# metagentools/VStrains

Measured on AMD Instinct MI355X. Metric: PE read pairs/sec through PE-link inference (GFA index + packed reads in HBM -> node_mat/short_mat), higher is better.
Workload: dtype u32

## Files before the change

### include/vstrains_hip.h

```cpp
#ifndef VSTRAINS_HIP_H
#define VSTRAINS_HIP_H

#include <stddef.h>
#include <stdint.h>

#ifdef __cplusplus
extern "C" {
#endif

#define VS_ABI_VERSION 10

enum {
    VS_OK = 0,
    VS_E_ARG = -1,
    VS_E_HIP = -2,
    VS_E_OOM = -3,
    VS_E_NODE_BASE = -4,
    VS_E_STATE = -5,
    VS_E_RANGE = -6,
    VS_E_UTF8 = -7,
    VS_E_KEY = -8,
    VS_E_FPE = -9,
    VS_E_RECURSION = -10
};
// ... 63 lines not shown
int vs_bgzf_shard_plan(const uint32_t *counts, uint64_t n_members, int no_final_newline, uint64_t first, uint64_t last, uint64_t plan[3]);
int vs_fastq_stream_open_range(vs_ctx *ctx, const char *fwd_path, const char *rve_path, const uint64_t range[6], uint64_t n_pairs,
                               vs_fastq_stream **out);

int vs_write_matrix_text(vs_ctx *ctx, const char *path, const uint8_t *ids, const uint64_t *id_off,
                         uint32_t n, const int64_t *mat);

int vs_synth_pairs(vs_ctx *ctx, const uint8_t *genomes, const uint64_t *goff,
                   const uint32_t *cum, uint32_t n_strains, uint64_t seed, uint64_t first_pair,
                   uint64_t n_pairs, uint32_t read_len, uint32_t sub_thresh, uint32_t n_thresh,
                   vs_reads **out);

int vs_pe_count(vs_ctx *ctx, const vs_reads *reads, uint32_t *d_node_mat, uint32_t *d_short_mat,
                uint64_t *d_stats);

int vs_pe_count_tracked(vs_ctx *ctx, const vs_reads *reads, uint32_t *d_node_mat, uint32_t *d_short_mat,
                        uint64_t *d_stats, uint8_t *d_tile_map);
int vs_counts_zero_tracked(vs_ctx *ctx, uint32_t *d_node_mat, uint32_t *d_short_mat, uint32_t n, uint8_t *d_tile_map);

int vs_counts_fold(vs_ctx *ctx, uint32_t *d_counts, int64_t *d_wide, uint64_t n);

int vs_counts_occupied(vs_ctx *ctx, const void *d_cells, uint32_t cell_bytes, uint64_t n_stretches, uint8_t *d_occ);

int vs_comm_unique_id(vs_ctx *ctx, uint8_t id[128]);
int vs_comm_init_rank(vs_ctx *ctx, int n_ranks, const uint8_t id[128], int rank, void **comm);
int vs_comm_destroy(vs_ctx *ctx, void *comm);
int vs_pe_allreduce(vs_ctx *ctx, void *comm, void *d_node_mat, void *d_short_mat, uint64_t *d_stats,
                    uint32_t n, int wide);

int vs_pe_map_ends(vs_ctx *ctx, const vs_reads *reads, uint32_t cap, uint32_t *lists,
                   uint32_t *counts);

int vs_pe_last_timing(vs_ctx *ctx, double ms[5]);
const char *vs_pe_last_kernel(const vs_ctx *ctx);
enum {
    VS_RAN_LOCUS_LDS_SORT = 1,
    VS_RAN_LOCUS_GLOBAL_SORT = 2,
    VS_RAN_PE_MID = 8,
    VS_RAN_ROW_OWNERS = 16
};
uint32_t vs_pe_last_launched(const vs_ctx *ctx);

typedef struct vs_links vs_links;
int vs_links_from_counts(vs_ctx *ctx, const uint32_t *d_node_mat, const uint32_t *d_short_mat,
                         uint32_t n, vs_links **out);
int vs_links_from_counts_tracked(vs_ctx *ctx, const uint32_t *d_node_mat, const uint32_t *d_short_mat, uint32_t n,
                                 const uint8_t *d_tile_map, uint32_t sparse_min_nodes, vs_links **out);
int vs_links_from_wide(vs_ctx *ctx, const int64_t *d_node_mat, const int64_t *d_short_mat,
                       uint32_t n, vs_links **out);
int vs_links_from_host(vs_ctx *ctx, const int64_t *node_mat, const int64_t *short_mat, uint32_t n,
                       vs_links **out);
int vs_links_reserve(vs_ctx *ctx, uint32_t n);
void vs_links_free(vs_ctx *ctx, vs_links *links);
int vs_links_size(const vs_links *links, uint32_t *n);
int vs_links_to_host(vs_ctx *ctx, const vs_links *links, int64_t *out );
int vs_links_block_sums(vs_ctx *ctx, const vs_links *links, const uint64_t *list_off,
                        const uint32_t *list_idx, uint32_t n_lists, const uint32_t *qa,
                        const uint32_t *qb, uint64_t n_queries, int64_t *out);
int vs_links_group_matrix(vs_ctx *ctx, const vs_links *links, const uint64_t *list_off,
                          const uint32_t *list_idx, uint32_t n_groups, int64_t *out);

int vs_graph_refresh(vs_ctx *ctx, uint32_t n_vertices, uint32_t n_edge_slots,
                     const uint64_t *row_ptr, const uint32_t *n_out, const uint32_t *nbr,
                     const uint32_t *eidx, const double *dp, const uint8_t *vertex_black,
                     const uint8_t *edge_black, double *flow, uint8_t *nontrivial,
                     uint8_t *fork_kind, int32_t *chain_next, int32_t *chain_top,
// ... 46 lines not shown
```

### vstrains_amd/_native.py

```python
from __future__ import annotations

import ctypes as C
import os

_HERE = os.path.dirname(os.path.abspath(__file__))
LIB_PATH = os.path.join(_HERE, "libvstrains_hip.so")

VS_OK = 0
VS_E_ARG, VS_E_HIP, VS_E_OOM, VS_E_NODE_BASE, VS_E_STATE, VS_E_RANGE, VS_E_UTF8, VS_E_KEY, VS_E_FPE = -1, -2, -3, -4, -5, -6, -7, -8, -9

SYMBOLS = {
    "vs_abi_version": (C.c_int, []),
    "vs_device_count": (C.c_int, []),
    "vs_ctx_create": (C.c_int, [C.c_int, C.POINTER(C.c_void_p)]),
    "vs_ctx_destroy": (None, [C.c_void_p]),
    "vs_last_error": (C.c_char_p, [C.c_void_p]),
    "vs_ctx_set_stream": (C.c_int, [C.c_void_p, C.c_void_p]),
    "vs_ctx_sync": (C.c_int, [C.c_void_p]),
    "vs_index_build": (C.c_int, [C.c_void_p, C.c_void_p, C.c_void_p, C.c_uint32, C.c_uint32,
                                 C.POINTER(C.c_uint32), C.POINTER(C.c_uint8)]),
    "vs_index_info": (C.c_int, [C.c_void_p, C.POINTER(C.c_uint64)]),
    "vs_index_export": (C.c_int, [C.c_void_p, C.c_void_p, C.c_void_p, C.c_void_p, C.c_void_p, C.c_void_p, C.POINTER(C.c_uint64)]),
    "vs_node_order_host": (C.c_int, [C.c_void_p, C.c_void_p, C.c_uint32, C.c_uint32, C.c_void_p]),
    "vs_reads_pack": (C.c_int, [C.c_void_p, C.c_void_p, C.c_void_p, C.c_uint64, C.POINTER(C.c_void_p)]),
# ... 13 lines not shown
    "vs_fastq_block": (C.c_int, [C.c_void_p, C.c_void_p, C.c_uint64, C.c_uint64, C.POINTER(C.c_void_p)]),
    "vs_fastq_stream_open": (C.c_int, [C.c_void_p, C.c_char_p, C.c_char_p, C.POINTER(C.c_void_p)]),
    "vs_fastq_stream_next": (C.c_int, [C.c_void_p, C.c_void_p, C.c_uint64, C.POINTER(C.c_void_p), C.POINTER(C.c_uint64)]),
    "vs_fastq_stream_info": (C.c_int, [C.c_void_p, C.POINTER(C.c_uint64)]),
    "vs_fastq_stream_close": (None, [C.c_void_p]),
    "vs_fastq_scan_text": (C.c_int, [C.c_void_p, C.c_void_p, C.c_uint64, C.c_uint32, C.c_void_p, C.c_uint64, C.POINTER(C.c_uint64)]),
    "vs_bgzf_walk": (C.c_int, [C.c_void_p, C.c_uint64, C.c_void_p, C.c_uint64, C.POINTER(C.c_uint64)]),
    "vs_inflate_host": (C.c_int, [C.c_void_p, C.c_uint32, C.c_void_p, C.c_uint32, C.c_uint32, C.POINTER(C.c_uint32)]),
    "vs_inflate_bgzf": (C.c_int, [C.c_void_p, C.c_void_p, C.c_uint64, C.c_void_p, C.c_uint64, C.c_uint32, C.c_void_p, C.c_uint64,
                                  C.POINTER(C.c_uint64)]),
    "vs_fastq_stream_inflate_info": (C.c_int, [C.c_void_p, C.POINTER(C.c_uint64)]),
    "vs_bgzf_walk_file": (C.c_int, [C.c_char_p, C.c_void_p, C.c_uint64, C.POINTER(C.c_uint64)]),
    "vs_bgzf_count_lines": (C.c_int, [C.c_void_p, C.c_char_p, C.c_void_p, C.c_uint64, C.c_void_p, C.POINTER(C.c_uint64)]),
    "vs_inflate_count_host": (C.c_int, [C.c_void_p, C.c_uint32, C.c_uint32, C.c_uint32, C.POINTER(C.c_uint32)]),
    "vs_bgzf_shard_plan": (C.c_int, [C.c_void_p, C.c_uint64, C.c_int, C.c_uint64, C.c_uint64, C.POINTER(C.c_uint64)]),
    "vs_fastq_stream_open_range": (C.c_int, [C.c_void_p, C.c_char_p, C.c_char_p, C.POINTER(C.c_uint64), C.c_uint64, C.POINTER(C.c_void_p)]),
    "vs_write_matrix_text": (C.c_int, [C.c_void_p, C.c_char_p, C.c_void_p, C.c_void_p, C.c_uint32, C.c_void_p]),
    "vs_synth_pairs": (C.c_int, [C.c_void_p, C.c_void_p, C.c_void_p, C.c_void_p, C.c_uint32, C.c_uint64,
                                 C.c_uint64, C.c_uint64, C.c_uint32, C.c_uint32, C.c_uint32,
                                 C.POINTER(C.c_void_p)]),
    "vs_pe_count": (C.c_int, [C.c_void_p, C.c_void_p, C.c_void_p, C.c_void_p, C.c_void_p]),
    "vs_pe_count_tracked": (C.c_int, [C.c_void_p, C.c_void_p, C.c_void_p, C.c_void_p, C.c_void_p, C.c_void_p]),
    "vs_counts_zero_tracked": (C.c_int, [C.c_void_p, C.c_void_p, C.c_void_p, C.c_uint32, C.c_void_p]),
    "vs_counts_fold": (C.c_int, [C.c_void_p, C.c_void_p, C.c_void_p, C.c_uint64]),
    "vs_counts_occupied": (C.c_int, [C.c_void_p, C.c_void_p, C.c_uint32, C.c_uint64, C.c_void_p]),
    "vs_comm_unique_id": (C.c_int, [C.c_void_p, C.c_void_p]),
    "vs_comm_init_rank": (C.c_int, [C.c_void_p, C.c_int, C.c_void_p, C.c_int, C.POINTER(C.c_void_p)]),
    "vs_comm_destroy": (C.c_int, [C.c_void_p, C.c_void_p]),
    "vs_pe_allreduce": (C.c_int, [C.c_void_p, C.c_void_p, C.c_void_p, C.c_void_p, C.c_void_p, C.c_uint32, C.c_int]),
    "vs_pe_map_ends": (C.c_int, [C.c_void_p, C.c_void_p, C.c_uint32, C.c_void_p, C.c_void_p]),
    "vs_pe_last_kernel": (C.c_char_p, [C.c_void_p]),
    "vs_pe_last_launched": (C.c_uint32, [C.c_void_p]),
    "vs_pe_last_timing": (C.c_int, [C.c_void_p, C.POINTER(C.c_double)]),
    "vs_links_from_counts": (C.c_int, [C.c_void_p, C.c_void_p, C.c_void_p, C.c_uint32, C.POINTER(C.c_void_p)]),
    "vs_links_from_counts_tracked": (C.c_int, [C.c_void_p, C.c_void_p, C.c_void_p, C.c_uint32, C.c_void_p, C.c_uint32, C.POINTER(C.c_void_p)]),
    "vs_links_from_wide": (C.c_int, [C.c_void_p, C.c_void_p, C.c_void_p, C.c_uint32, C.POINTER(C.c_void_p)]),
    "vs_links_from_host": (C.c_int, [C.c_void_p, C.c_void_p, C.c_void_p, C.c_uint32, C.POINTER(C.c_void_p)]),
    "vs_links_reserve": (C.c_int, [C.c_void_p, C.c_uint32]),
    "vs_links_free": (None, [C.c_void_p, C.c_void_p]),
    "vs_links_size": (C.c_int, [C.c_void_p, C.POINTER(C.c_uint32)]),
    "vs_links_to_host": (C.c_int, [C.c_void_p, C.c_void_p, C.c_void_p]),
    "vs_links_block_sums": (C.c_int, [C.c_void_p, C.c_void_p, C.c_void_p, C.c_void_p, C.c_uint32, C.c_void_p,
                                      C.c_void_p, C.c_uint64, C.c_void_p]),
    "vs_links_group_matrix": (C.c_int, [C.c_void_p, C.c_void_p, C.c_void_p, C.c_void_p, C.c_uint32, C.c_void_p]),
    "vs_graph_refresh": (C.c_int, [C.c_void_p, C.c_uint32, C.c_uint32] + [C.c_void_p] * 13 + [C.POINTER(C.c_uint32)]),
    "vs_stage_create": (C.c_int, [C.c_void_p, C.c_void_p, C.POINTER(C.c_void_p)]),
    "vs_dev_alloc": (C.c_int, [C.c_void_p, C.c_size_t, C.POINTER(C.c_void_p)]),
    "vs_dev_free": (C.c_int, [C.c_void_p, C.c_void_p]),
    "vs_dev_zero": (C.c_int, [C.c_void_p, C.c_void_p, C.c_size_t]),
    "vs_dev_to_host": (C.c_int, [C.c_void_p, C.c_void_p, C.c_void_p, C.c_size_t]),
}

_lib = None


class NativeError(RuntimeError):
    def __init__(self, code: int, msg: str):
        super().__init__("libvstrains_hip: %s (code %d)" % (msg, code))
        self.code = code


def lib():
    global _lib
    if _lib is None:
        if not os.path.exists(LIB_PATH):
            raise ImportError(
# ... 20 lines not shown
```

### vstrains_amd/csrc/vs_internal.h

```cpp
#pragma once

#include <hip/hip_runtime.h>
#include <stdint.h>
#include <string>
#include <vector>

#include "../../include/vstrains_hip.h"
#include "vs_buf.h"
#include "vs_pe_plan.h"

#define VS_WAVE 64
#define VS_PAD_WORDS 16


struct VsNodeMeta {
    uint32_t woff;
    uint32_t len;
};

struct VsSlot {
    uint64_t key;
    uint32_t a;
    uint32_t b;
};
// ... 46 lines not shown
    const uint32_t *inv4;
};
#define VS_FLAG_N 1u
#define VS_FLAG_INVALID 2u
#define VS_FLAG_MANY 4u
#define VS_LEN_MASK 0x00FFFFFFu

struct FqStage {
    VsPinnedBuf words, woff, meta;
    hipEvent_t done = nullptr;
    bool in_flight = false;
};

void vs_tuning_load(VsTuning &t, bool experiment);

struct vs_ctx {
    int device = 0;
    bool experiment = false;
    VsTuning tune;
    hipStream_t stream = nullptr;
    std::string err;
    FqStage fq_stage[2];
    unsigned fq_next = 0;
    bool has_index = false;
    VsIndexDev idx{};
    VsDevBuf d_meta, d_fwd, d_table, d_post;
    uint64_t n_seed_pos = 0, n_slots = 0, n_distinct = 0, index_bytes = 0;
    uint32_t max_node_len = 0;
    VsDevBuf d_slow_list;
    VsDevBuf d_slow_count;
    enum SlowCount : uint32_t {
        SC_MID = 0,
        SC_ACC_QUEUE = 1,
        SC_SLOW = 8,
        SC_STRIP_QUEUE = 9,
        SC_OWNERS = 15,
        SC_WORDS = 16
    };
    VsDevBuf links_spare;
    uint32_t links_spare_n = 0;
    VsDevBuf d_slow_list2;
    VsDevBuf d_dense;
    uint32_t dense_nodes = 0xFFFFFFFFu;
    VsDevBuf d_locus_keys, d_perm, d_locus_hist, d_scan_tmp;
    double last_sort_ms = 0;
    VsDevBuf d_lists, d_list_counts;
    VsDevBuf d_rows, d_row_entries, d_mult, d_ltab;
    VsDevBuf scratch[32];
    struct CachedBuf { VsDevBuf buf; bool used; };
    std::vector<CachedBuf> cache;
    hipEvent_t ev[5] = {nullptr, nullptr, nullptr, nullptr, nullptr};
    double last_ms[3] = {0, 0, 0};
    const char *last_kernel = "";
    uint32_t last_launched = 0;
    int n_cu = 256;
};

struct vs_reads {
    uint64_t n_ends = 0, n_words = 0, max_len = 0, n_invalid = 0, bytes = 0;
    void *d_woff = nullptr, *d_meta = nullptr, *d_words = nullptr, *d_mask = nullptr, *d_inv4 = nullptr;
    bool cached = false;
    VsDevBuf own[5];
    unsigned n_own = 0;
    hipError_t own_alloc(void *&view, size_t bytes) {
        const hipError_t e = own[n_own].reserve(bytes);
        view = own[n_own].ptr();
// ... 131 lines not shown
```

### vstrains_amd/csrc/vs_pe.hip

```cpp
#include <stdio.h>
#include <stdlib.h>
#include <string.h>

#include "vs_internal.h"

#define TPB 256
#define LCAP 20u
__device__ __forceinline__ const uint32_t *vs_row_quad(const uint32_t *__restrict__ lists, const uint32_t *__restrict__ hi, uint64_t row, uint32_t q) {
    return q < LC / 4u ? lists + row * LC + 4u * q : hi + row * 4u;
}
#define EMPTY_NODE 0xFFFFFFFFu

struct PeParams {
    VsIndexDev idx;
    VsReadsDev rd;
    uint32_t *node_mat, *short_mat;
    unsigned long long *stats;
    uint32_t ept, pmax, words_cap, pool, pool_bits;
    uint64_t n_tiles;
    uint32_t *slow_list, *slow_count;
    uint32_t *dbg_lists, *dbg_counts;
    uint32_t dbg_cap;
    uint32_t accumulate;
    const uint32_t *perm;
// ... 784 lines not shown
                for (uint32_t i = lt; i < total; i += TTPB) ol[i] = s_list[i];
                for (uint32_t i = lt; i < ne; i += TTPB) {
                    const uint32_t n = (s_state[i] & 3u) == 1u ? s_ns[i] : 0u;
                    P.out_counts[(uint64_t)tile * ept + i] = n ? n | (s_off[i] >> 2) << 8 : 0u;
                }
            } else {
                uint32_t *ol = P.out_lists + (uint64_t)tile * ept * LC, *oh = P.out_lists_hi + (uint64_t)tile * ept * 4u;
                for (uint32_t i = lt; i < ne * (LCAP / 4u); i += TTPB) {
                    const uint32_t e = i / (LCAP / 4u), q4 = 4u * (i - e * (LCAP / 4u));
                    const uint32_t n = (s_state[e] & 3u) == 1u ? s_ns[e] : 0u;
                    if (q4 < n) {
                        const uint32_t *src = s_list + s_off[e] + q4;
                        *(VsQuad *)(q4 < LC ? ol + e * LC + q4 : oh + e * 4u) = VsQuad{src[0], src[1], src[2], src[3]};
                    }
                }
                for (uint32_t i = lt; i < ne; i += TTPB)
                    P.out_counts[(uint64_t)tile * ept + i] = (s_state[i] & 3u) == 1u ? s_ns[i] : 0u;
            }
        }
        if (want_dbg) {
            for (uint32_t i = tid; i < ne; i += TTPB) {
                if (s_state[i] & 2u) continue;
                uint32_t n = s_ns[i];
                const uint64_t ge = s_gend[i];
                P.dbg_counts[ge] = n;
                for (uint32_t k2 = 0; k2 < n && k2 < P.dbg_cap; k2++) P.dbg_lists[ge * P.dbg_cap + k2] = s_list[s_off[i] + k2];
            }
        }
    }
    __syncthreads();
    if (tid < 3 && P.stats && s_misc[12 + tid]) atomicAdd(&P.stats[tid], (unsigned long long)s_misc[12 + tid]);
}

#define ACC_LDS_BYTES ((2u * ACC_SLOTS + (ACC_TPB / 64) * 66u + (LCAP + 1u) + (LCAP + 1u) * ACC_GMAX + 4u) * 4u)
#define ACC_RUN 4u
#define ACC_GMAX 60u
#define ACC_PPW 64u
template <uint32_t BITS>
struct CellTable {
    static constexpr uint32_t EMPTY = 0xFFFFFFFFu;
    __device__ static uint32_t key(uint32_t mat, uint32_t x, uint32_t y, uint32_t N) { return (mat * N + x) * N + y; }
    __device__ static uint32_t slot(uint32_t k) { return ((((k >> 4) * 0x9E3779B1u) >> (36u - BITS)) << 4) | (k & 15u); }
    __device__ static uint32_t next(uint32_t at) { return (at + 16u) & ((1u << BITS) - 1u); }
};
typedef CellTable<ACC_BITS> Acc32;

template <typename TB>
__device__ __forceinline__ bool vs_cell_claim(uint32_t *s_key, uint32_t *s_cnt, uint32_t *s_used, uint32_t key, uint32_t at, uint32_t wgt) {
    for (uint32_t pr = 0; pr < 8u; pr++) {
        uint32_t kx = s_key[at];
        if (kx == TB::EMPTY) {
            kx = atomicCAS(&s_key[at], TB::EMPTY, key);
            if (kx == TB::EMPTY) { atomicAdd(s_used, 1u); kx = key; }
        }
        if (kx == key) {
            atomicAdd(&s_cnt[at], wgt);
            return true;
        }
        at = TB::next(at);
    }
    return false;
}

__global__ void __launch_bounds__(ACC_TPB)
k_pe_accumulate(const uint32_t *__restrict__ lists, const uint32_t *__restrict__ counts, uint64_t n_slots_pairs,
                uint32_t pairs_per_wg, uint32_t N, uint32_t use_table, uint32_t fill_limit,
                uint32_t *__restrict__ node_mat, uint32_t *__restrict__ short_mat, uint32_t *__restrict__ queue, uint32_t ept) {
    uint32_t *s_key = vs_lds;
    uint32_t *s_cnt = vs_lds + ACC_SLOTS;
    uint32_t(*s_pref)[66] = (uint32_t(*)[66])(vs_lds + 2u * ACC_SLOTS);
    uint32_t *s_g = vs_lds + 2u * ACC_SLOTS + (ACC_TPB / 64) * 66u;
    uint32_t *s_ua = s_g + (LCAP + 1u);
    uint32_t &s_used = s_ua[(LCAP + 1u) * ACC_GMAX];
    uint32_t &s_lost = s_ua[(LCAP + 1u) * ACC_GMAX + 1u];
    const uint32_t tid = threadIdx.x, lane = tid & 63u, wv = tid >> 6;
    const uint32_t NN = N * N;
    for (uint32_t i = tid; i < ACC_SLOTS; i += ACC_TPB) { s_key[i] = Acc32::EMPTY; s_cnt[i] = 0; }
    if (tid <= LCAP) {
        uint32_t gsum = 0;
        for (uint32_t m = 1; m <= tid; m++) gsum += (m + ACC_RUN - 1u) / ACC_RUN;
        s_g[tid] = gsum;
        uint32_t r = 0;
        for (uint32_t a2 = 0; a2 < tid; a2++)
            for (uint32_t c = 0; c < (tid - a2 + ACC_RUN - 1u) / ACC_RUN; c++) s_ua[tid * ACC_GMAX + r++] = a2;
    }
    if (tid == 0) { s_used = 0; s_lost = 0; }
    __syncthreads();
    uint32_t &s_chunk = s_ua[(LCAP + 1u) * ACC_GMAX + 2u];
    const uint32_t ppt = ept >> 1, region_q = (ept * LC) >> 2;
    auto write_out = [&]() {
        for (uint32_t i = tid; i < ACC_SLOTS; i += ACC_TPB) {
            const uint32_t key = s_key[i];
            if (key != Acc32::EMPTY) {
                atomicAdd(key >= NN ? short_mat + (key - NN) : node_mat + key, s_cnt[i]);
                s_key[i] = Acc32::EMPTY;
                s_cnt[i] = 0;
            }
        }
        if (tid == 0) { s_used = 0; s_lost = 0; }
        __syncthreads();
    };
    for (;;) {
    __syncthreads();
    if (tid == 0) s_chunk = atomicAdd(queue, 1u);
    __syncthreads();
    const uint64_t chunk = s_chunk;
    const uint64_t lo = chunk * pairs_per_wg;
    if (lo >= n_slots_pairs) break;
    const uint64_t hi = lo + pairs_per_wg < n_slots_pairs ? lo + pairs_per_wg : n_slots_pairs;
    for (uint64_t base = lo; base < hi; base += (ACC_TPB / 64u) * ACC_PPW) {
        const uint64_t wbase = base + wv * ACC_PPW;
        const uint32_t *wcounts = counts + 2u * wbase;
        const uint64_t tile0 = wbase / ppt;
        const uint32_t rem0 = (uint32_t)(wbase - tile0 * ppt);
        const uint32_t *wlists = lists + tile0 * ept * LC;
        uint32_t nl = 0, nr = 0, packed = 0;
        if (wbase + lane < hi) {
            const uint2 c = *(const uint2 *)(wcounts + 2u * lane);
            nl = c.x & 0xFFu; nr = c.y & 0xFFu;
            const uint32_t tq = (rem0 + lane) / ppt * region_q;
            packed = nl | nr << 5 | (tq + (c.x >> 8)) << 10 | (tq + (c.y >> 8)) << 21;
        }
        const uint32_t u = nl * ((nr + ACC_RUN - 1u) / ACC_RUN) + s_g[nl] + s_g[nr];
        const uint32_t incl = vs_wave_scan_add(u);
        s_pref[wv][lane + 1u] = incl;
        if (lane == 0) s_pref[wv][0] = 0;
        if (lane == 63u) s_pref[wv][65] = 0xFFFFFFFFu;
        const uint32_t U = __shfl(incl, 63, 64);
        __builtin_amdgcn_fence(__ATOMIC_RELEASE, "workgroup");
        __builtin_amdgcn_wave_barrier();
        uint32_t cur = 0;
        struct Run {
            uint32_t x, mat, bi, be;
            VsQuad yq;
            bool ok;
        };
        auto fetch = [&](uint32_t t0) {
            Run R;
            while (s_pref[wv][cur + 1u] <= t0) cur++;
            const uint32_t t_raw = t0 + lane;
            const uint32_t t = t_raw < U ? t_raw : U - 1u;
            uint32_t a0 = cur;
            a0 += s_pref[wv][a0 + 1u] <= t ? 1u : 0u;
            a0 += s_pref[wv][a0 + 1u] <= t ? 1u : 0u;
            a0 += s_pref[wv][a0 + 1u] <= t ? 1u : 0u;
            while (s_pref[wv][a0 + 1u] <= t) a0++;
            uint32_t r = t - s_pref[wv][a0];
            const uint32_t pk = __shfl(packed, (int)a0, 64);
            const uint32_t ql = pk & 31u, qr = (pk >> 5) & 31u, rowl = ((pk >> 10) & 0x7FFu) << 2, rowr = (pk >> 21) << 2;
            R.ok = t_raw < U;
            const uint32_t cq = (qr + ACC_RUN - 1u) / ACC_RUN;
            uint32_t off;
            if (r < ql * cq) {
                const uint32_t a = cq == 1u ? r : cq == 2u ? r >> 1 : cq == 4u ? r >> 2 : cq == 3u ? (r * 43691u) >> 17 : (r * 52429u) >> 18;
                R.x = wlists[rowl + a]; R.mat = 0u; off = rowr; R.bi = ACC_RUN * (r - a * cq); R.be = qr;
            } else {
                r -= ql * cq;
                uint32_t n = ql;
                off = rowl;
                const uint32_t gl = s_g[ql];
                if (r >= gl) { r -= gl; n = qr; off = rowr; }
                const uint32_t a = s_ua[n * ACC_GMAX + r];
                const uint32_t crun = r - (s_g[n] - s_g[n - a]);
                R.x = wlists[off + a]; R.mat = 1u; R.bi = a + ACC_RUN * crun; R.be = n;
            }
            R.yq = *(const VsQuad *)(wlists + off + R.bi);
            return R;
        };
        Run nxt;
        nxt.ok = false;
        if (U) nxt = fetch(0u);
        for (uint32_t t0 = 0; t0 < U; t0 += 64u) {
            const Run c = nxt;
            if (t0 + 64u < U) nxt = fetch(t0 + 64u);
            if (!c.ok) continue;
            const uint32_t x = c.x, mat = c.mat, bi = c.bi, be = c.be;
            const uint32_t ys[ACC_RUN] = {c.yq.x, c.yq.y, c.yq.z, c.yq.w};
            if (use_table) {
                uint32_t key[ACC_RUN], seen[ACC_RUN], at[ACC_RUN];
#pragma unroll
                for (uint32_t j = 0; j < ACC_RUN; j++) {
                    const uint32_t yv = ys[j];
                    const uint32_t cx = (mat && yv < x) ? yv : x, cy = (mat && yv < x) ? x : yv;
                    key[j] = Acc32::key(mat, cx, cy, N);
                    at[j] = Acc32::slot(key[j]);
                    seen[j] = s_key[at[j]];
                }
#pragma unroll
                for (uint32_t j = 0; j < ACC_RUN; j++) {
                    if (bi + j >= be) continue;
                    if (seen[j] == key[j]) {
                        atomicAdd(&s_cnt[at[j]], 1u);
                    } else if (!vs_cell_claim<Acc32>(s_key, s_cnt, &s_used, key[j], at[j], 1u)) {
                        atomicAdd(&s_lost, 1u);
                        atomicAdd(key[j] >= NN ? short_mat + (key[j] - NN) : node_mat + key[j], 1u);
                    }
                }
            } else {
#pragma unroll
                for (uint32_t j = 0; j < ACC_RUN; j++) {
                    if (bi + j >= be) continue;
                    const uint32_t yv = ys[j];
                    const uint32_t cx = (mat && yv < x) ? yv : x, cy = (mat && yv < x) ? x : yv;
                    atomicAdd((mat ? short_mat : node_mat) + (uint64_t)cx * N + cy, 1u);
                }
            }
        }
        __syncthreads();
        const bool spill = s_used > fill_limit || s_lost > 4096u;
        __syncthreads();
        if (spill) write_out();
    }
    }
    __syncthreads();
    write_out();
}

__global__ void __launch_bounds__(256) k_mark_tiles(const uint32_t *__restrict__ lists, const uint32_t *__restrict__ counts,
                                                   uint64_t n_slots_pairs, uint8_t *__restrict__ map, uint32_t T, uint32_t ept) {
    const uint64_t p = (uint64_t)blockIdx.x * blockDim.x + threadIdx.x;
    if (p >= n_slots_pairs) return;
    const uint32_t cl = counts[2u * p], cr = counts[2u * p + 1u], nl = cl & 0xFFu, nr = cr & 0xFFu;
    if (!nl && !nr) return;
    const uint32_t *region = lists + 2u * p / ept * ept * LC, *rl = region + 4u * (cl >> 8), *rr = region + 4u * (cr >> 8);
    uint8_t *smap = map + (uint64_t)T * T;
    uint32_t tl[8], tr[8], kl = 0, kr = 0;
    bool over = false;
    auto put = [&](uint32_t (&tt)[8], uint32_t &k, uint32_t t) {
        bool seen = false;
#pragma unroll
        for (uint32_t j = 0; j < 8u; j++) seen |= j < k && tt[j] == t;
        if (seen) return;
        if (k >= 8u) { over = true; return; }
#pragma unroll
        for (uint32_t j = 0; j < 8u; j++)
            if (j == k) tt[j] = t;
        k++;
    };
// ... 1029 lines not shown
                               ctx->d_locus_hist.as<uint32_t>());
            int rc = vs_scan_u32(ctx, ctx->d_locus_hist.as<const uint32_t>(), ctx->d_locus_hist.as<uint32_t>(), nk,
                                 ctx->d_scan_tmp.as<uint64_t>(), nullptr);
            if (rc) return rc;
            hipLaunchKernelGGL(k_pe_permute, dim3(pg), dim3(TPB), 0, st, n_pairs, ctx->d_locus_keys.as<const uint32_t>(),
                               ctx->d_locus_hist.as<uint32_t>(), ctx->d_perm.as<uint32_t>());
        }
    }
    VS_HIP(ctx, hipEventRecord(ctx->ev[0], st));
    if (!d_node_mat) VS_HIP(ctx, hipEventRecord(ctx->ev[4], st));
    ctx->last_kernel = tf->name;
    {
        void *kargs[] = {(void *)&P};
        VS_HIP(ctx, hipLaunchKernel(tf->fn, dim3((unsigned)pl.grid), dim3(TTPB), kargs, lds, st));
    }
    if (d_node_mat) {
        const uint64_t used_ends = 2ull * n_pairs;
        if (pl.list_ends > used_ends)
            VS_HIP(ctx, hipMemsetAsync(ctx->d_list_counts.as<uint32_t>() + used_ends, 0, sizeof(uint32_t) * (pl.list_ends - used_ends), st));
        const uint64_t slots_pairs = pl.list_ends / 2;
        VS_HIP(ctx, hipEventRecord(ctx->ev[4], st));
        if (pl.use_rows) {
            const int rc = pe_count_by_rows(ctx, pl, d_node_mat, d_short_mat, d_tile_map, P.tile_T);
            if (rc) return rc;
            ctx->last_launched |= VS_RAN_ROW_OWNERS;
        } else {
            uint32_t *acc_queue = ctx->d_slow_count.as<uint32_t>() + vs_ctx::SC_ACC_QUEUE;
            if (pl.mark_tiles)
                hipLaunchKernelGGL(k_mark_tiles, dim3((unsigned)((slots_pairs + 255u) / 256u)), dim3(256), 0, st, ctx->d_lists.as<const uint32_t>(),
                                   ctx->d_list_counts.as<const uint32_t>(), slots_pairs, d_tile_map, P.tile_T, pl.ept);
            VS_HIP(ctx, hipFuncSetAttribute((const void *)k_pe_accumulate, hipFuncAttributeMaxDynamicSharedMemorySize, (int)ACC_LDS_BYTES));
            hipLaunchKernelGGL(k_pe_accumulate, dim3(pl.acc_grid), dim3(ACC_TPB), ACC_LDS_BYTES, st, ctx->d_lists.as<const uint32_t>(),
                               ctx->d_list_counts.as<const uint32_t>(), slots_pairs, pl.acc_per_wg, idx.n_nodes, pl.use_table, pl.acc_fill, d_node_mat,
                               d_short_mat, acc_queue, pl.ept);
        }
    }
    VS_HIP(ctx, hipEventRecord(ctx->ev[1], st));
    const bool no_mid = ctx->tune.no_mid;
    ctx->last_launched |= no_mid ? 0u : VS_RAN_PE_MID;
    if (!no_mid) {
        hipLaunchKernelGGL(k_pe_mid, dim3((unsigned)ctx->n_cu * 8u), dim3(TPB), 0, st, P, ctx->d_slow_list.as<const uint32_t>(),
                           ctx->d_slow_count.as<const uint32_t>(), (uint32_t)n_pairs, ctx->d_slow_list2.as<uint32_t>(), ctx->d_slow_count.as<uint32_t>() + vs_ctx::SC_SLOW);
        hipLaunchKernelGGL(k_pe_slow, dim3(pl.slow_grid), dim3(TPB), 0, st, P, ctx->d_dense.as<uint32_t>(), (uint32_t)n_pairs,
                           ctx->d_slow_list2.as<const uint32_t>(), ctx->d_slow_count.as<const uint32_t>() + vs_ctx::SC_SLOW);
    } else {
        hipLaunchKernelGGL(k_pe_slow, dim3(pl.slow_grid), dim3(TPB), 0, st, P, ctx->d_dense.as<uint32_t>(), (uint32_t)n_pairs,
                           ctx->d_slow_list.as<const uint32_t>(), ctx->d_slow_count.as<const uint32_t>());
    }
    VS_HIP(ctx, hipEventRecord(ctx->ev[2], st));
    VS_HIP(ctx, hipGetLastError());
    return VS_OK;
}

extern "C" int vs_pe_count(vs_ctx *ctx, const vs_reads *reads, uint32_t *d_node_mat, uint32_t *d_short_mat, uint64_t *d_stats) {
    if (!ctx || !reads || !d_node_mat || !d_short_mat || !d_stats) return VS_E_ARG;
    return pe_launch(ctx, reads, d_node_mat, d_short_mat, d_stats, nullptr, nullptr, 0);
}

extern "C" int vs_pe_count_tracked(vs_ctx *ctx, const vs_reads *reads, uint32_t *d_node_mat, uint32_t *d_short_mat, uint64_t *d_stats,
                                   uint8_t *d_tile_map) {
    if (!ctx || !reads || !d_node_mat || !d_short_mat || !d_stats || !d_tile_map) return VS_E_ARG;
    return pe_launch(ctx, reads, d_node_mat, d_short_mat, d_stats, nullptr, nullptr, 0, d_tile_map);
}

extern "C" int vs_counts_zero_tracked(vs_ctx *ctx, uint32_t *d_node_mat, uint32_t *d_short_mat, uint32_t n, uint8_t *d_tile_map) {
    if (!ctx || (n && (!d_node_mat || !d_short_mat || !d_tile_map))) return vs_fail(ctx, VS_E_ARG, "vs_counts_zero_tracked: bad argument");
    if (!n) return VS_OK;
    VS_HIP(ctx, hipSetDevice(ctx->device));
    const uint32_t T = (n + 63u) >> 6;
    const uint64_t tiles = 2ull * T * T;
    if (tiles > 0x7FFFFFFFull) return vs_fail(ctx, VS_E_RANGE, "vs_counts_zero_tracked: %u nodes make more tiles than one launch takes", n);
    hipLaunchKernelGGL(k_zero_tiles, dim3((unsigned)((tiles + 63u) / 64u)), dim3(64), 0, ctx->stream, d_node_mat, d_short_mat, n, T, d_tile_map, tiles);
    VS_HIP(ctx, hipGetLastError());
    return VS_OK;
}

extern "C" const char *vs_pe_last_kernel(const vs_ctx *ctx) { return ctx ? ctx->last_kernel : ""; }
extern "C" uint32_t vs_pe_last_launched(const vs_ctx *ctx) { return ctx ? ctx->last_launched : 0u; }

extern "C" int vs_pe_last_timing(vs_ctx *ctx, double ms[5]) {
    if (!ctx || !ms) return VS_E_ARG;
    VS_HIP(ctx, hipSetDevice(ctx->device));
    VS_HIP(ctx, hipEventSynchronize(ctx->ev[2]));
    float a = 0, b = 0, c = 0, d = 0;
    VS_HIP(ctx, hipEventElapsedTime(&a, ctx->ev[0], ctx->ev[1]));
    VS_HIP(ctx, hipEventElapsedTime(&d, ctx->ev[4], ctx->ev[1]));
    if (d > a) d = 0;
    a -= d;
    VS_HIP(ctx, hipEventElapsedTime(&b, ctx->ev[1], ctx->ev[2]));
    VS_HIP(ctx, hipEventElapsedTime(&c, ctx->ev[3], ctx->ev[0]));
    ctx->last_sort_ms = c;
    uint32_t n_slow = 0;
    VS_HIP(ctx, hipMemcpy(&n_slow, ctx->d_slow_count.ptr(), sizeof n_slow, hipMemcpyDeviceToHost));
    ms[0] = a; ms[1] = b; ms[2] = (double)n_slow; ms[3] = c; ms[4] = d;
    ctx->last_ms[0] = a; ctx->last_ms[1] = b; ctx->last_ms[2] = n_slow;
    return VS_OK;
}

extern "C" int vs_pe_map_ends(vs_ctx *ctx, const vs_reads *reads, uint32_t cap, uint32_t *lists, uint32_t *counts) {
    if (!ctx || !reads || !lists || !counts || !cap) return VS_E_ARG;
    VS_HIP(ctx, hipSetDevice(ctx->device));
    uint64_t n = reads->n_ends;
    if (!n) return VS_OK;
    VsDevBuf lists_buf, counts_buf;
    VS_HIP(ctx, lists_buf.reserve(sizeof(uint32_t) * n * cap));
    VS_HIP(ctx, counts_buf.reserve(sizeof(uint32_t) * n));
    uint32_t *d_lists = lists_buf.as<uint32_t>(), *d_counts = counts_buf.as<uint32_t>();
    VS_HIP(ctx, hipMemsetAsync(d_counts, 0, sizeof(uint32_t) * n, ctx->stream));
    VS_HIP(ctx, hipMemsetAsync(d_lists, 0xFF, sizeof(uint32_t) * n * cap, ctx->stream));
    const int rc = pe_launch(ctx, reads, nullptr, nullptr, nullptr, d_lists, d_counts, cap);
    if (rc != VS_OK) return rc;
    VS_HIP(ctx, hipMemcpyAsync(lists, d_lists, sizeof(uint32_t) * n * cap, hipMemcpyDeviceToHost, ctx->stream));
    VS_HIP(ctx, hipMemcpyAsync(counts, d_counts, sizeof(uint32_t) * n, hipMemcpyDeviceToHost, ctx->stream));
    VS_HIP(ctx, hipStreamSynchronize(ctx->stream));
    return rc;
}
```

### vstrains_amd/csrc/vs_pe_plan.h

```cpp
#ifndef VS_PE_PLAN_H
#define VS_PE_PLAN_H
#include <stddef.h>
#include <stdint.h>
#include <stdio.h>

#include <initializer_list>

#include "../../include/vstrains_hip.h"

#if defined(__HIPCC__)
#define VS_PLAN_FN __host__ __device__ inline
#else
#define VS_PLAN_FN inline
#endif

struct VsTuning {
    uint32_t ept = 0;
    uint32_t grid_per_cu = 128;
    int acc_fill_pct = -1;
    int shortcut = -1;
    int adapt_grid = -1;
    int acc_rows = -1;
    int ltab_bits = -1;
    uint32_t rows_keys = 0, rows_sub = 0;
    uint32_t rows_per_strip = 0;
    bool no_sort = false, locus_global = false, no_fast = false, no_std = false, no_agg = false;
    bool no_mid = false;
};

VS_PLAN_FN uint32_t vs_seed_phase(uint32_t len, uint32_t w, uint32_t s) {
    return len < w ? 0u : ((len - w) % s + s) / 2u;
}
VS_PLAN_FN uint32_t vs_seed_probes(uint32_t len, uint32_t w, uint32_t s) {
    if (len < w) return 0u;
    return (len - w + 1u) / s;
}
#define VS_SEED_VERIFIED(w) ((w) <= 31u ? (w) : 0u)

#define LC 16u
#define PPT 2u
#define TTPB 256
#define PPT_LONG 1u
#define CHUNK (TTPB * PPT)
#define ACC_TPB 1024
#define ACC_BITS 14
#define ACC_SLOTS (1u << ACC_BITS)
#define ROWS_KEYS 65536u
#define ROWS_SUB ((1u << 26) - 1024u)
#define RS_BITS 13
#define RS_SLOTS (1u << RS_BITS)
#define LOCUS_LDS_KEYS 36864u
#define LOCUS_LDS_MAX_PASSES 4u
#define LOCUS_WGS 256u
#define SLOW_WORDS_PER_NODE 6u
#define LDS_BUDGET_BYTES (64u * 1024u)
#define NI_CAP 4096u

struct TileLayout {
    uint32_t woff, gend, meta, inv, words, pcnt, pa, pb, hkey, hcnt, hminp, hminj, ns, state, list, owner, misc, total;
};
VS_PLAN_FN TileLayout tile_layout(uint32_t ept, uint32_t pmax, uint32_t words_cap, uint32_t pool, uint32_t list_trim = 0u) {
    TileLayout t;
    uint32_t o = 0;
    const uint32_t NI = ept * pmax;
    t.woff = o;  o += 2u * ((ept + 2u) & ~1u);
    t.gend = o;  o += 2u * ept;
    t.meta = o;  o += 2u * ept;
    t.inv = o;   o += ept;
    t.words = o; o += 2u * (words_cap + 8u);
    t.pcnt = o;  o += NI + 1u;
    t.pa = o;    o += NI;
    t.pb = o;    o += NI;
    t.hkey = o;  o += pool;
    t.hcnt = o;  o += pool;
    t.hminp = o; o += pool;
    t.hminj = o; o += pool;
    t.ns = o;    o += ept;
    t.state = o; o += ept;
    t.list = o;
// ... 197 lines not shown
```

### vstrains_amd/pe.py

```python
from __future__ import annotations

import ctypes as C
import os
from typing import List, Optional, Sequence, Tuple

import numpy as np

from . import _native as nat
from .dist import U32_LIMIT, ExchangeState


def _universal_newlines(raw: bytes) -> bytes:
    if b"\r" in raw:
        raw = raw.replace(b"\r\n", b"\n").replace(b"\r", b"\n")
    return raw


def read_gfa_segments(path: str) -> Tuple[List[str], List[str]]:
    with open(path, "rb") as fh:
        raw = _universal_newlines(fh.read())
    ids: List[str] = []
    seqs: List[str] = []
    pieces = raw.split(b"\n")
    last_has_nl = raw.endswith(b"\n")
# ... 575 lines not shown

    def pack_pairs(self, fwd: Sequence[str], rve: Sequence[str]) -> ReadBlock:
        n = min(len(fwd), len(rve))
        seqs: List[str] = []
        for r in range(n):
            seqs.append(fwd[r])
            seqs.append(rve[r])
        data, off = encode_seqs(seqs)
        return self.pack(data, off)

    def synth_pairs(self, genomes: Sequence[str], cum: np.ndarray, seed: int, first_pair: int, n_pairs: int,
                    read_len: int, sub_thresh: int = 0, n_thresh: int = 0) -> ReadBlock:
        gd, go = encode_seqs(genomes)
        cum = np.ascontiguousarray(cum, dtype=np.uint32)
        h = C.c_void_p()
        nat.check(self._h, nat.lib().vs_synth_pairs(self._h, gd.ctypes.data, go.ctypes.data, cum.ctypes.data,
                                                    len(genomes), seed, first_pair, n_pairs, read_len,
                                                    sub_thresh, n_thresh, C.byref(h)))
        return ReadBlock(self, h)

    def pe_count(self, reads: ReadBlock, node_mat_ptr: int, short_mat_ptr: int, stats_ptr: int, tile_map_ptr: Optional[int] = None):
        if tile_map_ptr is not None:
            nat.check(self._h, nat.lib().vs_pe_count_tracked(self._h, reads._h, C.c_void_p(node_mat_ptr), C.c_void_p(short_mat_ptr),
                                                             C.c_void_p(stats_ptr), C.c_void_p(tile_map_ptr)))
            return
        nat.check(self._h, nat.lib().vs_pe_count(self._h, reads._h, C.c_void_p(node_mat_ptr),
                                                 C.c_void_p(short_mat_ptr), C.c_void_p(stats_ptr)))

    def last_timing(self):
        a = (C.c_double * 5)()
        nat.check(self._h, nat.lib().vs_pe_last_timing(self._h, a))
        return dict(main_ms=a[0], slow_ms=a[1], slow_pairs=int(a[2]), sort_ms=a[3], accumulate_ms=a[4])

    @property
    def last_kernel(self) -> str:
        return (nat.lib().vs_pe_last_kernel(self._h) or b"").decode()

    RAN_LOCUS_LDS_SORT, RAN_LOCUS_GLOBAL_SORT, RAN_PE_MID, RAN_ROW_OWNERS = 1, 2, 8, 16

    @property
    def last_launched(self) -> int:
        return int(nat.lib().vs_pe_last_launched(self._h))

    def map_ends(self, reads: ReadBlock, cap: int = 64) -> List[List[int]]:
        n = reads.info["ends"]
        lists = np.zeros((max(n, 1), cap), dtype=np.uint32)
        counts = np.zeros(max(n, 1), dtype=np.uint32)
        nat.check(self._h, nat.lib().vs_pe_map_ends(self._h, reads._h, cap, lists.ctypes.data, counts.ctypes.data))
        out = []
        for e in range(n):
            c = int(counts[e])
            if c > cap:
                raise ValueError("end %d has %d nodes, cap %d" % (e, c, cap))
            ids = lists[e, :c] if self.node_order is None else self.node_order[lists[e, :c]]
            out.append(sorted(int(x) for x in ids))
        return out


class PeCounter:

    TRACK_TILES_MIN_BYTES = 2 << 30

    def __init__(self, ctx: Context, device: Optional[str] = None, track_tiles: Optional[bool] = None):
        import torch

        self.torch = torch
# ... 169 lines not shown
```

Before: 1.355 billion.

## Deduplicate node pairs per 32-pair group via wave-local hash tables with bitmasks

The accumulate kernel used to expand every pair's left/right node lists into individual (x,y) cells and add 1 per cell. It now inserts the nodes of 32 pairs into a per-wave LDS hash table, each node carrying a bitmask of the pairs that hit it. It then enumerates distinct node pairs and adds popcount(maskA & maskB) once per cell, so repeated cells across pairs cost one table update instead of many. When the small table overflows the group is halved and retried, and a counter records these halvings. The cost is extra LDS, wave barriers and compaction work, which may not pay off when node lists are sparse or rarely overlap.

```diff
diff --git a/include/vstrains_hip.h b/include/vstrains_hip.h
--- a/include/vstrains_hip.h
+++ b/include/vstrains_hip.h
@@ -119,6 +119,8 @@
                    uint32_t *counts);
 
 int vs_pe_last_timing(vs_ctx *ctx, double ms[5]);
+
+int vs_pe_acc_halvings(vs_ctx *ctx, uint32_t *n);
 const char *vs_pe_last_kernel(const vs_ctx *ctx);
 enum {
     VS_RAN_LOCUS_LDS_SORT = 1,
diff --git a/vstrains_amd/_native.py b/vstrains_amd/_native.py
--- a/vstrains_amd/_native.py
+++ b/vstrains_amd/_native.py
@@ -69,6 +69,7 @@
     "vs_pe_last_kernel": (C.c_char_p, [C.c_void_p]),
     "vs_pe_last_launched": (C.c_uint32, [C.c_void_p]),
     "vs_pe_last_timing": (C.c_int, [C.c_void_p, C.POINTER(C.c_double)]),
+    "vs_pe_acc_halvings": (C.c_int, [C.c_void_p, C.POINTER(C.c_uint32)]),
     "vs_links_from_counts": (C.c_int, [C.c_void_p, C.c_void_p, C.c_void_p, C.c_uint32, C.POINTER(C.c_void_p)]),
     "vs_links_from_counts_tracked": (C.c_int, [C.c_void_p, C.c_void_p, C.c_void_p, C.c_uint32, C.c_void_p, C.c_uint32, C.POINTER(C.c_void_p)]),
     "vs_links_from_wide": (C.c_int, [C.c_void_p, C.c_void_p, C.c_void_p, C.c_uint32, C.POINTER(C.c_void_p)]),
diff --git a/vstrains_amd/csrc/vs_internal.h b/vstrains_amd/csrc/vs_internal.h
--- a/vstrains_amd/csrc/vs_internal.h
+++ b/vstrains_amd/csrc/vs_internal.h
@@ -102,6 +102,7 @@
     enum SlowCount : uint32_t {
         SC_MID = 0,
         SC_ACC_QUEUE = 1,
+        SC_ACC_HALVINGS = 2,
         SC_SLOW = 8,
         SC_STRIP_QUEUE = 9,
         SC_OWNERS = 15,
diff --git a/vstrains_amd/csrc/vs_pe.hip b/vstrains_amd/csrc/vs_pe.hip
--- a/vstrains_amd/csrc/vs_pe.hip
+++ b/vstrains_amd/csrc/vs_pe.hip
@@ -840,10 +840,16 @@
     if (tid < 3 && P.stats && s_misc[12 + tid]) atomicAdd(&P.stats[tid], (unsigned long long)s_misc[12 + tid]);
 }
 
-#define ACC_LDS_BYTES ((2u * ACC_SLOTS + (ACC_TPB / 64) * 66u + (LCAP + 1u) + (LCAP + 1u) * ACC_GMAX + 4u) * 4u)
-#define ACC_RUN 4u
-#define ACC_GMAX 60u
+#define ACC_WL (1u << ACC_WL_BITS)
+#define ACC_WR (1u << ACC_WR_BITS)
+#define ACC_WSLOTS (ACC_WL + ACC_WR)
+#define ACC_WAVE_WORDS (2u * ACC_WSLOTS + ACC_WQ / 2u)
+#define ACC_LDS_BYTES ((2u * ACC_SLOTS + 4u + (ACC_TPB / 64) * ACC_WAVE_WORDS) * 4u)
 #define ACC_PPW 64u
+static_assert(ACC_G == 32u, "a pair's bit lives in a 32-bit mask");
+static_assert(ACC_WSLOTS <= 256u && ACC_WQ >= 128u && (ACC_WQ & (ACC_WQ - 1u)) == 0u, "a ring entry is two 8-bit slot indices; 63 waiting entries + 64 new ones");
+static_assert(ACC_WL >= LCAP && ACC_WL <= 64u && ACC_WR == 2u * 64u, "one pair always fits; the compaction reads a lane per left slot and two per right slot");
+static_assert(ACC_LDS_BYTES <= 160u * 1024u, "k_pe_accumulate: LDS");
 template <uint32_t BITS>
 struct CellTable {
     static constexpr uint32_t EMPTY = 0xFFFFFFFFu;
@@ -870,31 +876,57 @@
     return false;
 }
 
+__device__ __forceinline__ void vs_wave_lds_sync() {
+    __builtin_amdgcn_fence(__ATOMIC_RELEASE, "workgroup");
+    __builtin_amdgcn_wave_barrier();
+    __builtin_amdgcn_fence(__ATOMIC_ACQUIRE, "workgroup");
+}
+
+__device__ __forceinline__ bool vs_wave_insert(uint32_t *wK, uint32_t *wM, uint32_t base, uint32_t bits, uint32_t node, uint32_t bit,
+                                               uint32_t limit) {
+    const uint32_t msk = (1u << bits) - 1u;
+    uint32_t h = (node * 0x9E3779B1u) >> (32u - bits);
+    for (uint32_t pr = 0; pr < limit; pr++) {
+        uint32_t kx = wK[base + h];
+        if (kx == Acc32::EMPTY) {
+            kx = atomicCAS(&wK[base + h], Acc32::EMPTY, node);
+            if (kx == Acc32::EMPTY) kx = node;
+        }
+        if (kx == node) {
+            atomicOr(&wM[base + h], bit);
+            return true;
+        }
+        h = (h + 1u) & msk;
+    }
+    return false;
+}
+
 __global__ void __launch_bounds__(ACC_TPB)
 k_pe_accumulate(const uint32_t *__restrict__ lists, const uint32_t *__restrict__ counts, uint64_t n_slots_pairs,
                 uint32_t pairs_per_wg, uint32_t N, uint32_t use_table, uint32_t fill_limit,
-                uint32_t *__restrict__ node_mat, uint32_t *__restrict__ short_mat, uint32_t *__restrict__ queue, uint32_t ept) {
+                uint32_t *__restrict__ node_mat, uint32_t *__restrict__ short_mat, uint32_t *__restrict__ queue, uint32_t ept,
+                uint32_t *__restrict__ halvings) {
     uint32_t *s_key = vs_lds;
     uint32_t *s_cnt = vs_lds + ACC_SLOTS;
-    uint32_t(*s_pref)[66] = (uint32_t(*)[66])(vs_lds + 2u * ACC_SLOTS);
-    uint32_t *s_g = vs_lds + 2u * ACC_SLOTS + (ACC_TPB / 64) * 66u;
-    uint32_t *s_ua = s_g + (LCAP + 1u);
-    uint32_t &s_used = s_ua[(LCAP + 1u) * ACC_GMAX];
-    uint32_t &s_lost = s_ua[(LCAP + 1u) * ACC_GMAX + 1u];
+    uint32_t *s_misc = vs_lds + 2u * ACC_SLOTS;
+    uint32_t &s_used = s_misc[0];
+    uint32_t &s_lost = s_misc[1];
+    uint32_t &s_chunk = s_misc[2];
     const uint32_t tid = threadIdx.x, lane = tid & 63u, wv = tid >> 6;
+    uint32_t *wK = s_misc + 4u + wv * ACC_WAVE_WORDS;
+    uint32_t *wM = wK + ACC_WSLOTS;
+    uint16_t *wQ = (uint16_t *)(wM + ACC_WSLOTS);
     const uint32_t NN = N * N;
+    const unsigned long long lanes_below = (1ull << lane) - 1ull;
     for (uint32_t i = tid; i < ACC_SLOTS; i += ACC_TPB) { s_key[i] = Acc32::EMPTY; s_cnt[i] = 0; }
-    if (tid <= LCAP) {
-        uint32_t gsum = 0;
-        for (uint32_t m = 1; m <= tid; m++) gsum += (m + ACC_RUN - 1u) / ACC_RUN;
-        s_g[tid] = gsum;
-        uint32_t r = 0;
-        for (uint32_t a2 = 0; a2 < tid; a2++)
-            for (uint32_t c = 0; c < (tid - a2 + ACC_RUN - 1u) / ACC_RUN; c++) s_ua[tid * ACC_GMAX + r++] = a2;
-    }
+    auto wave_clear = [&]() {
+        vs_wave_lds_sync();
+        for (uint32_t i = lane; i < ACC_WSLOTS; i += 64u) { wK[i] = Acc32::EMPTY; wM[i] = 0u; }
+        vs_wave_lds_sync();
+    };
+    wave_clear();
     if (tid == 0) { s_used = 0; s_lost = 0; }
     __syncthreads();
-    uint32_t &s_chunk = s_ua[(LCAP + 1u) * ACC_GMAX + 2u];
     const uint32_t ppt = ept >> 1, region_q = (ept * LC) >> 2;
     auto write_out = [&]() {
         for (uint32_t i = tid; i < ACC_SLOTS; i += ACC_TPB) {
@@ -907,6 +939,59 @@
         }
         if (tid == 0) { s_used = 0; s_lost = 0; }
         __syncthreads();
+    };
+    uint32_t head = 0, tail = 0;
+    auto add_cells = [&](uint32_t cnt) {
+        vs_wave_lds_sync();
+        if (lane < cnt) {
+            const uint32_t e = wQ[(head + lane) & (ACC_WQ - 1u)], a = e >> 8, b = e & 255u;
+            const uint32_t x = wK[a], y = wK[b], wgt = (uint32_t)__popc(wM[a] & wM[b]);
+            const uint32_t mat = (a < ACC_WL && b >= ACC_WL) ? 0u : 1u;
+            const uint32_t cx = (mat && y < x) ? y : x, cy = (mat && y < x) ? x : y;
+            if (use_table) {
+                const uint32_t key = Acc32::key(mat, cx, cy, N), at = Acc32::slot(key);
+                if (s_key[at] == key) {
+                    atomicAdd(&s_cnt[at], wgt);
+                } else if (!vs_cell_claim<Acc32>(s_key, s_cnt, &s_used, key, at, wgt)) {
+                    atomicAdd(&s_lost, 1u);
+                    atomicAdd(key >= NN ? short_mat + (key - NN) : node_mat + key, wgt);
+                }
+            } else {
+                atomicAdd((mat ? short_mat : node_mat) + (uint64_t)cx * N + cy, wgt);
+            }
+        }
+        head += cnt;
+    };
+    auto push = [&](bool hit, uint32_t a, uint32_t b) {
+        const unsigned long long bal = __ballot(hit);
+        if (!bal) return;
+        if (hit) wQ[(tail + (uint32_t)__popcll(bal & lanes_below)) & (ACC_WQ - 1u)] = (uint16_t)(a << 8 | b);
+        tail += (uint32_t)__popcll(bal);
+        if (tail - head >= 64u) add_cells(64u);
+    };
+    auto rect = [&](uint32_t a0, uint32_t na, uint32_t b0, uint32_t nb, bool tri) {
+        const uint32_t total = na * nb;
+        if (!total) return;
+        const float rcp = 1.0f / (float)nb;
+        for (uint32_t t0 = 0; t0 < total; t0 += 64u) {
+            const uint32_t t_raw = t0 + lane, t = t_raw < total ? t_raw : total - 1u;
+            const uint32_t i = (uint32_t)(((float)t + 0.5f) * rcp), j = t - i * nb;
+            const uint32_t a = a0 + i, b = b0 + j;
+            const bool hit = t_raw < total && (!tri || i <= j) && (wM[a] & wM[b]) != 0u;
+            push(hit, a, b);
+        }
+    };
+    auto fold = [&](uint32_t a0, uint32_t n) {
+        for (uint32_t i = 0; 2u * i < n; i++) {
+            const uint32_t i2 = n - 1u - i, len1 = n - i, total = i2 == i ? len1 : n + 1u;
+            for (uint32_t c0 = 0; c0 < total; c0 += 64u) {
+                const uint32_t c_raw = c0 + lane, c = c_raw < total ? c_raw : 0u;
+                const bool first = c < len1;
+                const uint32_t a = a0 + (first ? i : i2), b = a0 + (first ? i + c : i2 + (c - len1));
+                const bool hit = c_raw < total && (wM[a] & wM[b]) != 0u;
+                push(hit, a, b);
+            }
+        }
     };
     for (;;) {
     __syncthreads();
@@ -922,96 +1007,57 @@
         const uint64_t tile0 = wbase / ppt;
         const uint32_t rem0 = (uint32_t)(wbase - tile0 * ppt);
         const uint32_t *wlists = lists + tile0 * ept * LC;
-        uint32_t nl = 0, nr = 0, packed = 0;
+        uint32_t cl = 0, cr = 0;
         if (wbase + lane < hi) {
             const uint2 c = *(const uint2 *)(wcounts + 2u * lane);
-            nl = c.x & 0xFFu; nr = c.y & 0xFFu;
             const uint32_t tq = (rem0 + lane) / ppt * region_q;
-            packed = nl | nr << 5 | (tq + (c.x >> 8)) << 10 | (tq + (c.y >> 8)) << 21;
-        }
-        const uint32_t u = nl * ((nr + ACC_RUN - 1u) / ACC_RUN) + s_g[nl] + s_g[nr];
-        const uint32_t incl = vs_wave_scan_add(u);
-        s_pref[wv][lane + 1u] = incl;
-        if (lane == 0) s_pref[wv][0] = 0;
-        if (lane == 63u) s_pref[wv][65] = 0xFFFFFFFFu;
-        const uint32_t U = __shfl(incl, 63, 64);
-        __builtin_amdgcn_fence(__ATOMIC_RELEASE, "workgroup");
-        __builtin_amdgcn_wave_barrier();
-        uint32_t cur = 0;
-        struct Run {
-            uint32_t x, mat, bi, be;
-            VsQuad yq;
-            bool ok;
-        };
-        auto fetch = [&](uint32_t t0) {
-            Run R;
-            while (s_pref[wv][cur + 1u] <= t0) cur++;
-            const uint32_t t_raw = t0 + lane;
-            const uint32_t t = t_raw < U ? t_raw : U - 1u;
-            uint32_t a0 = cur;
-            a0 += s_pref[wv][a0 + 1u] <= t ? 1u : 0u;
-            a0 += s_pref[wv][a0 + 1u] <= t ? 1u : 0u;
-            a0 += s_pref[wv][a0 + 1u] <= t ? 1u : 0u;
-            while (s_pref[wv][a0 + 1u] <= t) a0++;
-            uint32_t r = t - s_pref[wv][a0];
-            const uint32_t pk = __shfl(packed, (int)a0, 64);
-            const uint32_t ql = pk & 31u, qr = (pk >> 5) & 31u, rowl = ((pk >> 10) & 0x7FFu) << 2, rowr = (pk >> 21) << 2;
-            R.ok = t_raw < U;
-            const uint32_t cq = (qr + ACC_RUN - 1u) / ACC_RUN;
-            uint32_t off;
-            if (r < ql * cq) {
-                const uint32_t a = cq == 1u ? r : cq == 2u ? r >> 1 : cq == 4u ? r >> 2 : cq == 3u ? (r * 43691u) >> 17 : (r * 52429u) >> 18;
-                R.x = wlists[rowl + a]; R.mat = 0u; off = rowr; R.bi = ACC_RUN * (r - a * cq); R.be = qr;
-            } else {
-                r -= ql * cq;
-                uint32_t n = ql;
-                off = rowl;
-                const uint32_t gl = s_g[ql];
-                if (r >= gl) { r -= gl; n = qr; off = rowr; }
-                const uint32_t a = s_ua[n * ACC_GMAX + r];
-                const uint32_t crun = r - (s_g[n] - s_g[n - a]);
-                R.x = wlists[off + a]; R.mat = 1u; R.bi = a + ACC_RUN * crun; R.be = n;
-            }
-            R.yq = *(const VsQuad *)(wlists + off + R.bi);
-            return R;
-        };
-        Run nxt;
-        nxt.ok = false;
-        if (U) nxt = fetch(0u);
-        for (uint32_t t0 = 0; t0 < U; t0 += 64u) {
-            const Run c = nxt;
-            if (t0 + 64u < U) nxt = fetch(t0 + 64u);
-            if (!c.ok) continue;
-            const uint32_t x = c.x, mat = c.mat, bi = c.bi, be = c.be;
-            const uint32_t ys[ACC_RUN] = {c.yq.x, c.yq.y, c.yq.z, c.yq.w};
-            if (use_table) {
-                uint32_t key[ACC_RUN], seen[ACC_RUN], at[ACC_RUN];
-#pragma unroll
-                for (uint32_t j = 0; j < ACC_RUN; j++) {
-                    const uint32_t yv = ys[j];
-                    const uint32_t cx = (mat && yv < x) ? yv : x, cy = (mat && yv < x) ? x : yv;
-                    key[j] = Acc32::key(mat, cx, cy, N);
-                    at[j] = Acc32::slot(key[j]);
-                    seen[j] = s_key[at[j]];
-                }
-#pragma unroll
-                for (uint32_t j = 0; j < ACC_RUN; j++) {
-                    if (bi + j >= be) continue;
-                    if (seen[j] == key[j]) {
-                        atomicAdd(&s_cnt[at[j]], 1u);
-                    } else if (!vs_cell_claim<Acc32>(s_key, s_cnt, &s_used, key[j], at[j], 1u)) {
-                        atomicAdd(&s_lost, 1u);
-                        atomicAdd(key[j] >= NN ? short_mat + (key[j] - NN) : node_mat + key[j], 1u);
+            cl = (c.x & 0xFFu) | (tq + (c.x >> 8)) << 8;
+            cr = (c.y & 0xFFu) | (tq + (c.y >> 8)) << 8;
+        }
+        for (uint32_t g = 0; g < ACC_PPW / ACC_G; g++) {
+            const uint32_t pi = lane & (ACC_G - 1u), end = lane / ACC_G, src = g * ACC_G + pi;
+            const uint32_t wl = (uint32_t)__shfl((int)cl, (int)src, 64), wr = (uint32_t)__shfl((int)cr, (int)src, 64);
+            const uint32_t cw = end ? wr : wl, n = cw & 0xFFu;
+            if (!__ballot(n != 0u)) continue;
+            const uint32_t *row = wlists + 4u * (cw >> 8);
+            const uint32_t bit = 1u << pi, tb = end ? ACC_WL : 0u, tbits = end ? ACC_WR_BITS : ACC_WL_BITS;
+            uint32_t s = 0, len = ACC_G;
+            while (s < ACC_G) {
+                const bool in = pi >= s && pi < s + len;
+                const uint32_t limit = len == 1u ? ACC_WR : 24u;
+                bool fail = false;
+                for (uint32_t q = 0; __ballot(in && 4u * q < n); q++) {
+                    if (in && 4u * q < n) {
+                        const VsQuad v = *(const VsQuad *)(row + 4u * q);
+                        const uint32_t e[4] = {v.x, v.y, v.z, v.w};
+#pragma unroll
+                        for (uint32_t j = 0; j < 4u; j++)
+                            if (4u * q + j < n) fail |= !vs_wave_insert(wK, wM, tb, tbits, e[j], bit, limit);
                     }
                 }
-            } else {
-#pragma unroll
-                for (uint32_t j = 0; j < ACC_RUN; j++) {
-                    if (bi + j >= be) continue;
-                    const uint32_t yv = ys[j];
-                    const uint32_t cx = (mat && yv < x) ? yv : x, cy = (mat && yv < x) ? x : yv;
-                    atomicAdd((mat ? short_mat : node_mat) + (uint64_t)cx * N + cy, 1u);
-                }
+                vs_wave_lds_sync();
+                if (__ballot(fail) && len > 1u) {
+                    wave_clear();
+                    if (lane == 0) atomicAdd(halvings, 1u);
+                    len >>= 1;
+                    continue;
+                }
+                const uint32_t k0 = wK[lane], k1 = wK[ACC_WL + lane], k2 = wK[ACC_WL + 64u + lane];
+                const uint32_t m0 = wM[lane], m1 = wM[ACC_WL + lane], m2 = wM[ACC_WL + 64u + lane];
+                const unsigned long long b0 = __ballot(lane < ACC_WL && k0 != Acc32::EMPTY), b1 = __ballot(k1 != Acc32::EMPTY),
+                                         b2 = __ballot(k2 != Acc32::EMPTY);
+                const uint32_t nL = (uint32_t)__popcll(b0), c1 = (uint32_t)__popcll(b1), nR = c1 + (uint32_t)__popcll(b2);
+                vs_wave_lds_sync();
+                if ((b0 >> lane) & 1ull) { const uint32_t r = (uint32_t)__popcll(b0 & lanes_below); wK[r] = k0; wM[r] = m0; }
+                if ((b1 >> lane) & 1ull) { const uint32_t r = ACC_WL + (uint32_t)__popcll(b1 & lanes_below); wK[r] = k1; wM[r] = m1; }
+                if ((b2 >> lane) & 1ull) { const uint32_t r = ACC_WL + c1 + (uint32_t)__popcll(b2 & lanes_below); wK[r] = k2; wM[r] = m2; }
+                vs_wave_lds_sync();
+                rect(0u, nL, ACC_WL, nR, false);
+                if (nL <= 32u) rect(0u, nL, 0u, nL, true); else fold(0u, nL);
+                if (nR <= 32u) rect(ACC_WL, nR, ACC_WL, nR, true); else fold(ACC_WL, nR);
+                while (tail != head) add_cells(tail - head < 64u ? tail - head : 64u);
+                wave_clear();
+                s += len;
             }
         }
         __syncthreads();
@@ -2107,7 +2153,7 @@
             VS_HIP(ctx, hipFuncSetAttribute((const void *)k_pe_accumulate, hipFuncAttributeMaxDynamicSharedMemorySize, (int)ACC_LDS_BYTES));
             hipLaunchKernelGGL(k_pe_accumulate, dim3(pl.acc_grid), dim3(ACC_TPB), ACC_LDS_BYTES, st, ctx->d_lists.as<const uint32_t>(),
                                ctx->d_list_counts.as<const uint32_t>(), slots_pairs, pl.acc_per_wg, idx.n_nodes, pl.use_table, pl.acc_fill, d_node_mat,
-                               d_short_mat, acc_queue, pl.ept);
+                               d_short_mat, acc_queue, pl.ept, ctx->d_slow_count.as<uint32_t>() + vs_ctx::SC_ACC_HALVINGS);
         }
     }
     VS_HIP(ctx, hipEventRecord(ctx->ev[1], st));
@@ -2172,6 +2218,16 @@
     return VS_OK;
 }
 
+extern "C" int vs_pe_acc_halvings(vs_ctx *ctx, uint32_t *n) {
+    if (!ctx || !n) return VS_E_ARG;
+    *n = 0;
+    if (!ctx->d_slow_count.ptr()) return VS_OK;
+    VS_HIP(ctx, hipSetDevice(ctx->device));
+    VS_HIP(ctx, hipStreamSynchronize(ctx->stream));
+    VS_HIP(ctx, hipMemcpy(n, ctx->d_slow_count.as<uint32_t>() + vs_ctx::SC_ACC_HALVINGS, sizeof *n, hipMemcpyDeviceToHost));
+    return VS_OK;
+}
+
 extern "C" int vs_pe_map_ends(vs_ctx *ctx, const vs_reads *reads, uint32_t cap, uint32_t *lists, uint32_t *counts) {
     if (!ctx || !reads || !lists || !counts || !cap) return VS_E_ARG;
     VS_HIP(ctx, hipSetDevice(ctx->device));
diff --git a/vstrains_amd/csrc/vs_pe_plan.h b/vstrains_amd/csrc/vs_pe_plan.h
--- a/vstrains_amd/csrc/vs_pe_plan.h
+++ b/vstrains_amd/csrc/vs_pe_plan.h
@@ -45,6 +45,10 @@
 #define ACC_TPB 1024
 #define ACC_BITS 14
 #define ACC_SLOTS (1u << ACC_BITS)
+#define ACC_G 32u
+#define ACC_WL_BITS 6u
+#define ACC_WR_BITS 7u
+#define ACC_WQ 128u
 #define ROWS_KEYS 65536u
 #define ROWS_SUB ((1u << 26) - 1024u)
 #define RS_BITS 13
diff --git a/vstrains_amd/pe.py b/vstrains_amd/pe.py
--- a/vstrains_amd/pe.py
+++ b/vstrains_amd/pe.py
@@ -631,6 +631,11 @@
         nat.check(self._h, nat.lib().vs_pe_last_timing(self._h, a))
         return dict(main_ms=a[0], slow_ms=a[1], slow_pairs=int(a[2]), sort_ms=a[3], accumulate_ms=a[4])
 
+    def acc_halvings(self) -> int:
+        n = C.c_uint32(0)
+        nat.check(self._h, nat.lib().vs_pe_acc_halvings(self._h, C.byref(n)))
+        return int(n.value)
+
     @property
     def last_kernel(self) -> str:
         return (nat.lib().vs_pe_last_kernel(self._h) or b"").decode()
```

Result: slower. 1.034 billion (-23.7%).
